# ishine/TargetDiarization

Hardware: AMD Instinct MI355X
Metric: real-time factor (audio-sec/wall-sec) full infer() pipe, 16kHz mono, 1/2/4/8 GPU (higher is better)
Workload: dtype f32 (split-f16 x3: fp32-accurate products from three f16 MFMA passes, fp32 accumulate); 1 GPU; BASELINE configs[3]: 1800 s synthetic conversation (two alternating speakers, 20 % overlap) = 180 x 10 s windows: MossFormer2 (90 windows per launch) -> loudness swap -> ERes2NetV2 on every 10 s window of both streams + cosine vs a target embedding -> Paraformer (SANM encoder, CIF predictor, NAR decoder, argmax tokens + timestamps) on 30 s segments of both streams -> CT-Transformer punctuation of ; windows_per_launch=90

## Files before the change

targetdiarization_amd/csrc/eres2net.hip:

```cpp
#include <hip/hip_runtime.h>

#include <algorithm>
#include <cmath>
#include <string>
#include <vector>

#include "../../include/tdx.h"
#include "gemm.hpp"
#include "gemm_h3.hpp"
#include "devutil.hpp"
#include "tdx_common.hpp"

using namespace tdx;

namespace {

constexpr int NSTAGE = 4, SCALE = 4, EMB = 192;
const int kBlocks[NSTAGE] = {3, 4, 6, 3};
const int kPlanes[NSTAGE] = {64, 128, 256, 512};
const int kStride[NSTAGE] = {1, 2, 2, 2};

inline size_t al(size_t n) { return (n + 63) / 64 * 64; }
inline int up(int n, int m) { return (n + m - 1) / m * m; }

// ... 77 lines not shown
    __device__ EpiNone row(int, int) const { return EpiNone{}; }
    __device__ void store(int z, int m, int n, float v, EpiNone, EpiNone) const { slab[(long)z * strideZ + (long)m * (int)ld + n] = v; }
};
__global__ __launch_bounds__(256) void slab_reduce_kernel(const float* __restrict__ slab, int nz, long MN, int N, const float* __restrict__ bias, float* __restrict__ out) {
    const long i = ((long)blockIdx.x * 256 + threadIdx.x) * 4;
    if (i >= MN) return;
    float4 a = *reinterpret_cast<const float4*>(slab + i);
    for (int z = 1; z < nz; ++z) {
        const float4 p = *reinterpret_cast<const float4*>(slab + (long)z * MN + i);
        a.x += p.x; a.y += p.y; a.z += p.z; a.w += p.w;
    }
    if (bias) { const float4 b = *reinterpret_cast<const float4*>(bias + (int)(i % N)); a.x += b.x; a.y += b.y; a.z += b.z; a.w += b.w; }
    *reinterpret_cast<float4*>(out + i) = a;
}
struct EpiChain {
    const float* b; float* cat; long ldcat; int coff; int width; int wpad;
    const float* o1; long ldo1; int next_off; float* spin;
    __device__ float col(int, int n) const { return b[n]; }
    __device__ EpiNone row(int, int) const { return EpiNone{}; }
    __device__ float aux(int, int m, int n, EpiNone) const { return (spin && n < width) ? o1[(long)m * (int)ldo1 + next_off + n] : 0.f; }
    __device__ void store(int, int m, int n, float v, EpiNone, float c, float nxt) const {
        if (n >= wpad) return;
        const float sp = relu20(v + c);
        if (n < width) cat[(long)m * (int)ldcat + coff + n] = sp;
        if (spin) spin[(long)m * wpad + n] = n < width ? sp + nxt : 0.f;
    }
};
struct EpiConv3 {
    const float* b; const float* res; float* out; long ld;
    __device__ float col(int, int n) const { return b[n]; }
    __device__ EpiNone row(int, int) const { return EpiNone{}; }
    __device__ float aux(int, int m, int n, EpiNone) const { return res[(long)m * (int)ld + n]; }
    __device__ void store(int, int m, int n, float v, EpiNone, float c, float r) const { out[(long)m * (int)ld + n] = relu20(v + c + r); }
};
struct EpiAffSilu {
    const float* b; float* t; int ipad;
    __device__ float col(int, int n) const { return b[n]; }
    __device__ EpiNone row(int, int) const { return EpiNone{}; }
    __device__ void store(int, int m, int n, float v, EpiNone, float c) const { if (n < ipad) t[(long)m * ipad + n] = siluf_acc(v + c); }
};
struct EpiAffGate {
    const float* b; const float* x; long ldx; const float* y; long ldy; float* out; long ldo; int C;
    __device__ float col(int, int n) const { return b[n]; }
    __device__ EpiNone row(int, int) const { return EpiNone{}; }
    __device__ float2 aux(int, int m, int n, EpiNone) const {
        return n < C ? make_float2(x[(long)m * (int)ldx + n], y[(long)m * (int)ldy + n]) : make_float2(0.f, 0.f);
    }
    __device__ void store(int, int m, int n, float v, EpiNone, float c, float2 xy) const {
        if (n >= C) return;
        const float att = 1.0f + tanhf(v + c);
        out[(long)m * (int)ldo + n] = xy.x * att + xy.y * (2.0f - att);
    }
};


struct ChainX3Args {
    const float* in; long ldin;
    const unsigned char* wp; const float* ws; int wk;
    int cinp;
    const float* b;
    float* cat; long ldcat; int coff;
    const float* o1; long ldo1; int next_off; float* spin; int ldspin;
    int H, W;
};
template <int CIN, int TH>
struct ChainX3Cfg {
// ... 529 lines not shown
                if (s < 1) { for (int j = 0; j < SCALE; ++j) jobs.push_back(&b.convs[j]); continue; }
                jobs.push_back(&b.conv1); if (b.has_sc) jobs.push_back(&b.sc);
                for (int j = 0; j < SCALE; ++j) jobs.push_back(&b.convs[j]);
                jobs.push_back(&b.conv3);
            }
        jobs.push_back(&h->ds);
        jobs.push_back(&h->fuse34.c0); jobs.push_back(&h->fuse34.c3);
        size_t bytes = 0;
        for (ConvW* c : jobs) bytes += (size_t)c->Npad * c->taps * c->cinp * 4 + al(c->Npad) * 4;
        e = hipMalloc(&h->dev_planes, bytes);
        if (e != hipSuccess) { hipFree(h->dev); delete h; return tdx::fail_hip(e, __FILE__, __LINE__); }
        unsigned char* q = h->dev_planes;
        for (ConvW* c : jobs) {
            const int K = c->taps * c->cinp;
            float* sc = (float*)(q + (size_t)c->Npad * K * 4);
            e = tdx::launch_h3_split_rows_long(h->dev + c->w, K, q, sc, c->Npad, K, nullptr);
            if (e != hipSuccess) { hipFree(h->dev_planes); hipFree(h->dev); delete h; return tdx::fail_hip(e, __FILE__, __LINE__); }
            c->hp = q; c->hs = sc;
            q += (size_t)c->Npad * K * 4 + al(c->Npad) * 4;
        }
        e = hipDeviceSynchronize();
        if (e != hipSuccess) { hipFree(h->dev_planes); hipFree(h->dev); delete h; return tdx::fail_hip(e, __FILE__, __LINE__); }
    }
    *out = h;
    return TDX_OK;
}

int tdx_eres2net_destroy(tdx_eres2net* h) {
    if (h) { if (h->dev_planes) hipFree(h->dev_planes); if (h->dev) hipFree(h->dev); delete h; }
    return TDX_OK;
}

namespace {
struct WsPlan { size_t P, keep3, o1, spin, tbuf, stats, hx, hcat, hin, slab, total; };
inline WsPlan ws_plan(const tdx_eres2net* h, int B, int F) {
    const Dims d = make_dims(F);
    WsPlan w{}; size_t mP = (size_t)B * 80 * F * 64, mo1 = 0, msp = 0, mt = 0, mhx = 0, mhc = 0, mhi = 0;
    int s = 0, cnt = 0;
    for (const BlockW& b : h->blocks) {
        const size_t rows = (size_t)B * d.H[s + 1] * d.W[s + 1];
        if (s >= 1) {
            const size_t rows_in = cnt == 0 ? (size_t)B * d.H[s] * d.W[s] : rows;
            mhx = std::max(mhx, rows_in * b.cin); mhc = std::max(mhc, rows * b.w4); mhi = std::max(mhi, rows * b.wpad);
        }
        mP = std::max(mP, rows * b.cout); mo1 = std::max(mo1, rows * b.w4); msp = std::max(msp, rows * b.wpad);
        if (b.is_aff) mt = std::max(mt, rows * (size_t)b.aff[0].ipad);
        if (++cnt == kBlocks[s]) { cnt = 0; ++s; }
    }
    const size_t rows3 = (size_t)B * d.H[3] * d.W[3], rows4 = (size_t)B * d.H[4] * d.W[4];
    mt = std::max(mt, rows4 * 512);
    w.P = al(mP + 4096); w.keep3 = al(rows3 * 1024 + 4096); w.o1 = al(mo1 + 4096); w.spin = al(msp + 4096); w.tbuf = al(mt + 4096);
    w.stats = al((size_t)B * 40960);
    mhx = std::max(mhx, rows3 * 1024);
    w.hx = al(mhx + 4096); w.hcat = al(mhc + 4096); w.hin = al(mhi + 4096);
    w.slab = rows4 <= (size_t)DS_SPLIT_ROWS ? al(DS_SPLIT * rows4 * 2048 + 4096) : 0;
    w.total = 3 * w.P + w.keep3 + 2 * w.o1 + 2 * w.spin + w.tbuf + w.stats + w.hx + w.hcat + w.hin + w.slab;
    return w;
}
}

size_t tdx_eres2net_workspace_bytes(const tdx_eres2net* h, int B, int F) {
    if (!h || B < 1 || F < 9) return 0;
    return ws_plan(h, B, F).total * sizeof(float);
}

double tdx_eres2net_flops(const tdx_eres2net* h, int B, int F) {
    if (!h || F < 1) return 0.0;
    const Dims d = make_dims(F);
    double fl = 2.0 * 80 * F * 9 * 64;
    int s = 0, cnt = 0;
    for (const BlockW& b : h->blocks) {
        const double pos = (double)d.H[s + 1] * d.W[s + 1];
        fl += 2.0 * pos * ((double)b.cin * b.w4 + 4.0 * 9 * b.width * b.width + (double)b.w4 * b.cout + (b.has_sc ? (double)b.cin * b.cout : 0.0));
        if (b.is_aff) fl += 3.0 * 2.0 * pos * (2.0 * b.width * (b.width / 4) + (double)(b.width / 4) * b.width);
        if (++cnt == kBlocks[s]) { cnt = 0; ++s; }
    }
    const double pos4 = (double)d.H[4] * d.W[4];
    fl += 2.0 * pos4 * (9.0 * 1024 * 2048 + 4096.0 * 512 + 512.0 * 2048) + 2.0 * 40960 * EMB;
    return fl * B;
}

int tdx_eres2net_forward(tdx_eres2net* h, const float* feat, int B, int F, float* emb, void* ws_, size_t ws_bytes, void* stream) {
    if (!h || !feat || !emb || !ws_ || B < 1) return tdx::fail(TDX_E_INVALID, "tdx_eres2net_forward: bad argument");
    if (F < 9) return tdx::fail(TDX_E_INVALID, "tdx_eres2net_forward: need >= 9 fbank frames (TSTP needs >= 2 pooled frames)");
    const WsPlan wp = ws_plan(h, B, F);
    if (ws_bytes < wp.total * sizeof(float)) return tdx::fail(TDX_E_WORKSPACE, "tdx_eres2net_forward: workspace too small");
    tdx::DeviceGuard guard(h->device);
    if (guard.err != hipSuccess) return tdx::fail_hip(guard.err, __FILE__, __LINE__);
    hipStream_t st = (hipStream_t)stream;
    const Dims d = make_dims(F);
    const size_t rows1 = (size_t)B * 80 * F;
    float* ws = (float*)ws_;
    float* P[3] = {ws, ws + wp.P, ws + 2 * wp.P};
    float* keep3 = ws + 3 * wp.P;
    float* o1 = keep3 + wp.keep3; float* cat = o1 + wp.o1;
    float* spin[2] = {cat + wp.o1, cat + wp.o1 + wp.spin};
    float* tbuf = spin[1] + wp.spin; float* stats = tbuf + wp.tbuf;
    unsigned char* hx = (unsigned char*)(stats + wp.stats);
    unsigned char* hcat = hx + wp.hx * sizeof(float);
    unsigned char* hin = hcat + wp.hcat * sizeof(float);
    float* slab = reinterpret_cast<float*>(hin + wp.hin * sizeof(float));
    const float* inv20 = h->dev + h->consts;
    const float* inv40 = h->dev + h->consts + 1;
    const unsigned char* zero_row = (const unsigned char*)(h->dev + h->consts + 64);

    hipLaunchKernelGGL(stem_kernel, dim3((unsigned)((rows1 * 16 + 255) / 256)), dim3(256), 0, st, feat, h->dev + h->stem_w, h->dev + h->stem_b, P[0], F, (long)rows1);
    LAUNCH_CHECK();
    const float* x = P[0];
    int cur = 0;
    int s = 0, cnt = 0;
    for (const BlockW& b : h->blocks) {
        const int Hin = (cnt == 0) ? d.H[s] : d.H[s + 1], Win = (cnt == 0) ? d.W[s] : d.W[s + 1];
        const int Ho = d.H[s + 1], Wo = d.W[s + 1];
        const long M = (long)B * Ho * Wo;
        const bool last_of_stage3 = (s == 2) && (cnt == kBlocks[2] - 1);
        const int iy = cur < 0 ? 0 : (cur + 1) % 3, ir = cur < 0 ? 1 : (cur + 2) % 3;
        float* y = last_of_stage3 ? keep3 : P[iy];
        float* res = P[ir];
        const bool x3 = b.conv1.hp != nullptr;
        const float* resid = x;
        if (x3) {
            int Hc = Hin, Wc = Win, sc_ = b.stride;
            if (b.stride == 2 && b.cin % 16 == 0) {
                const long R = (long)B * Ho * Wo;
                hipLaunchKernelGGL(split_rows_static_s2_kernel, dim3((unsigned)((R * (b.cin / 8) + 255) / 256)), dim3(256), 0, st,
                                   x, b.cin, hx, R, b.cin, Hin, Win, Ho, Wo, 1024.0f);
                LAUNCH_CHECK();
                Hc = Ho; Wc = Wo; sc_ = 1;
            } else if (tdx::launch_h3_split_rows_static(x, b.cin, hx, (long)B * Hin * Win, b.cin, 1024.0f, st) != hipSuccess)
                return tdx::fail_hip(hipGetLastError(), __FILE__, __LINE__);
            TRY(conv_gemm_h3(hx, inv20, zero_row, b.conv1, B, Hc, Wc, Ho, Wo, sc_, EpiRelu20{h->dev + b.conv1.b, o1, b.w4, b.w4}, st));
            if (b.has_sc) {
                TRY(conv_gemm_h3(hx, inv20, zero_row, b.sc, B, Hc, Wc, Ho, Wo, sc_, EpiBiasG{h->dev + b.sc.b, res, b.cout, b.cout}, st));
                resid = res;
            }
        } else {
            TRY(conv_gemm(x, b.cin, h->dev, b.conv1, B, Hin, Win, Ho, Wo, b.stride, EpiRelu20{h->dev + b.conv1.b, o1, b.w4, b.w4}, st));
            if (b.has_sc) {
                TRY(conv_gemm(x, b.cin, h->dev, b.sc, B, Hin, Win, Ho, Wo, b.stride, EpiBiasG{h->dev + b.sc.b, res, b.cout, b.cout}, st));
                resid = res;
            }
        }
        for (int j = 0; j < SCALE; ++j) {
            const float* in = j == 0 ? o1 : spin[j & 1];
            const long ldin = j == 0 ? b.w4 : b.wpad;
            const bool plain_next = (j + 1 < SCALE) && !b.is_aff;
            EpiChain e{h->dev + b.convs[j].b, cat, b.w4, j * b.width, b.width, b.wpad, o1, b.w4, (j + 1) * b.width,
                       plain_next ? spin[(j + 1) & 1] : nullptr};
            if (b.convs[j].hp && !b.is_aff && (b.width == 24 || b.width == 48)) {
                ChainX3Args ca{in, ldin, b.convs[j].hp, b.convs[j].hs, 9 * b.convs[j].cinp, b.convs[j].cinp, h->dev + b.convs[j].b, cat, b.w4, j * b.width,
                               o1, b.w4, (j + 1) * b.width, plain_next ? spin[(j + 1) & 1] : nullptr, b.wpad, Ho, Wo};
                if (b.width == 24) TRY((launch_chain_x3<24, 4>(ca, B, st)));
                else TRY((launch_chain_x3<48, 4>(ca, B, st)));
            } else if (x3) {
                if (tdx::launch_h3_split_rows_static(in, ldin, hin, M, b.wpad, 512.0f, st) != hipSuccess)
                    return tdx::fail_hip(hipGetLastError(), __FILE__, __LINE__);
                TRY(conv_gemm_h3(hin, inv40, zero_row, b.convs[j], B, Ho, Wo, Ho, Wo, 1, e, st));
            } else {
                TRY(conv_gemm(in, ldin, h->dev, b.convs[j], B, Ho, Wo, Ho, Wo, 1, e, st));
            }
            if (b.is_aff && j + 1 < SCALE)
                TRY(run_aff(h, b.aff[j], cat + j * b.width, b.w4, o1 + (j + 1) * b.width, b.w4, tbuf, spin[(j + 1) & 1], b.wpad, M, st));
        }
        if (x3) {
            if (tdx::launch_h3_split_rows_static(cat, b.w4, hcat, M, b.w4, 1024.0f, st) != hipSuccess)
                return tdx::fail_hip(hipGetLastError(), __FILE__, __LINE__);
            TRY(conv_gemm_h3(hcat, inv20, zero_row, b.conv3, B, Ho, Wo, Ho, Wo, 1, EpiConv3{h->dev + b.conv3.b, resid, y, b.cout}, st));
        } else {
            GemmArgs g = make_args((int)M, b.conv3.Npad, make_seg(cat, b.w4, h->dev + b.conv3.w, b.conv3.cinp, b.conv3.cinp));
            if (launch_gemm<false, false, false, false>(g, 1, EpiConv3{h->dev + b.conv3.b, resid, y, b.cout}, st) != hipSuccess)
                return tdx::fail_hip(hipGetLastError(), __FILE__, __LINE__);
        }
        x = y;
        cur = last_of_stage3 ? -1 : iy;
        if (++cnt == kBlocks[s]) { cnt = 0; ++s; }
    }
    const int i_ds = (cur + 1) % 3, i_fu = (cur + 2) % 3;
    const long M4 = (long)B * d.H[4] * d.W[4];
    if (tdx::launch_h3_split_rows_static(keep3, 1024, hx, (long)B * d.H[3] * d.W[3], 1024, 1024.0f, st) != hipSuccess)
        return tdx::fail_hip(hipGetLastError(), __FILE__, __LINE__);
    if (wp.slab && h->ds.taps == 9 && h->ds.Npad == 2048)
        TRY(conv_gemm_h3_tapsplit(hx, inv20, zero_row, h->ds, B, d.H[3], d.W[3], d.H[4], d.W[4], 2, slab, nullptr, P[i_ds], st));
    else
        TRY(conv_gemm_h3(hx, inv20, zero_row, h->ds, B, d.H[3], d.W[3], d.H[4], d.W[4], 2, EpiBiasG{nullptr, P[i_ds], 2048, 2048}, st));
    const char* aff34_env = getenv("TDX_ERES_AFF34_ROWS");
    const long aff34_min = aff34_env ? atol(aff34_env) : 8192;
    if (M4 >= aff34_min && 2 * M4 <= (long)B * 40960 && h->fuse34.c0.hp && h->fuse34.ipad == 512)
        TRY(run_aff34_x3(h, h->fuse34, x, P[i_ds], tbuf, P[i_fu], M4, hx, hcat, stats, hin, stats + M4, inv20, st));
    else
        TRY(run_aff(h, h->fuse34, x, 2048, P[i_ds], 2048, tbuf, P[i_fu], 2048, M4, st));
    hipLaunchKernelGGL(tstp_kernel, dim3(d.H[4], B), dim3(256), 0, st, P[i_fu], stats, d.W[4], 2048, d.H[4]);
    LAUNCH_CHECK();
    hipLaunchKernelGGL(seg_kernel, dim3(EMB, B), dim3(256), 0, st, stats, h->dev + h->seg_w, h->dev + h->seg_b, emb, 40960);
    LAUNCH_CHECK();
    return TDX_OK;
}

}
```

targetdiarization_amd/csrc/gemm_h3.hpp:

```cpp
#pragma once
#include <cstdio>
#include <cstdlib>
#include <typeinfo>
#include <vector>
#include <hip/hip_runtime.h>
#include <stdint.h>

#include "devutil.hpp"
#include "gemm.hpp"

namespace tdx {

typedef _Float16 f16x8 __attribute__((ext_vector_type(8)));

constexpr int H3_BM = 256, H3_BN = 256, H3_BK = 16, H3_THREADS = 512;
constexpr int H3_ROWB = 64;
constexpr int H3_OPER = 256 * H3_ROWB;
constexpr int H3_STAGE = 2 * H3_OPER;
constexpr int H3_NBUF = 4;
constexpr int H3_AUX_AHEAD = 3;
constexpr int H3_LDS = H3_NBUF * H3_STAGE;
constexpr int H3_LDS_EXTRA = 12288;

struct H3Seg {
// ... 223 lines not shown
    for (int j = 0; j < 4; ++j) { const _Float16 t = (_Float16)xs[j]; a[j] = t; b[j] = (_Float16)(xs[j] - (float)t); }
    H3Pair r;
    r.hi = __builtin_bit_cast(uint2, a); r.lo = __builtin_bit_cast(uint2, b);
    return r;
}
__device__ __forceinline__ uint4 h3_pair16(int q, float4 v, float s) {
    const H3Pair o = h3_split4(v, s);
    const bool odd = q & 1;
    const uint2 send = odd ? o.hi : o.lo;
    uint2 recv;
    recv.x = (unsigned)__builtin_amdgcn_mov_dpp((int)send.x, 0xB1, 0xF, 0xF, true);
    recv.y = (unsigned)__builtin_amdgcn_mov_dpp((int)send.y, 0xB1, 0xF, 0xF, true);
    return odd ? make_uint4(recv.x, recv.y, o.lo.x, o.lo.y) : make_uint4(o.hi.x, o.hi.y, recv.x, recv.y);
}
__device__ __forceinline__ void h3_emit4(unsigned char* prow, int q, float4 v, float s) {
    *reinterpret_cast<uint4*>(prow + (q >> 1) * 32 + ((q & 1) ? 16 : 0)) = h3_pair16(q, v, s);
}
__device__ __forceinline__ void h3_emit4_pred(unsigned char* prow, int q, float4 v, float s, bool ok) {
    const uint4 w = h3_pair16(q, v, s);
    if (ok) *reinterpret_cast<uint4*>(prow + (q >> 1) * 32 + ((q & 1) ? 16 : 0)) = w;
}
__device__ __forceinline__ float h3_wave_max(float v) {
    v = h3_row16_max(v);
    return fmaxf(fmaxf(h3_lane(v, 0), h3_lane(v, 16)), fmaxf(h3_lane(v, 32), h3_lane(v, 48)));
}
__device__ __forceinline__ float h3_absmax4(float4 v) { return fmaxf(fmaxf(fabsf(v.x), fabsf(v.y)), fmaxf(fabsf(v.z), fabsf(v.w))); }


struct H3PlOut { unsigned char* planes; long pitch; float* scale; float* ss; long seg_stride; };
template <class E, class = void> struct epi_has_plout { static constexpr bool value = false; };
template <class E> struct epi_has_plout<E, decltype((void)&E::plout, void())> { static constexpr bool value = true; };
template <class E, class = void> struct epi_has_rowout { static constexpr bool value = false; };
template <class E> struct epi_has_rowout<E, decltype((void)&E::rowout, void())> { static constexpr bool value = true; };
struct H3Conv {
    const float* w; int wld;
    int ncols;
    unsigned char* planes; long pitch;
    float sv;
    float* u32; int u0; long ld32;
    int S, Sp;
};
template <class E, class = void> struct epi_has_conv { static constexpr bool value = false; };
template <class E> struct epi_has_conv<E, decltype((void)&E::conv, void())> { static constexpr bool value = true; };
constexpr int H3_CONV_STEP = 240, H3_CONV_HALO = 8;
template <class T> __device__ __forceinline__ void h3_assume_row(const T&) {}
__device__ __forceinline__ void h3_assume_row(long rw) { __builtin_assume(rw >= 0); }

template <bool A_TR, bool B_TR, bool PAIRED, bool TWOSEG, class Epi, int VARIANT = 0, bool A_CONV = false>
__global__ __launch_bounds__(H3_THREADS, 2) void gemm_h3_kernel(H3Args g, Epi epi) {
    static_assert(!A_CONV || (!A_TR && !TWOSEG), "A_CONV: row-major A planes, one weight segment");
    constexpr bool PINGPONG = VARIANT == 5;
    extern __shared__ __attribute__((aligned(1024))) unsigned char lds[];
    const int tid = threadIdx.x;
    const int lane = tid & 63, wave = tid >> 6;
    const int l31 = lane & 31, h = lane >> 5;
    const int wm = wave >> 2, wn = wave & 3;

    int z, bm, bn;
    {
        const int x = blockIdx.x & 7, i = blockIdx.x >> 3;
        if (g.map_mode == 0) {
            z = blockIdx.y;
            int i2 = i, mbase = 0, mcur = g.mp;
            if (g.mc > 0) { const int tpc = g.mc * g.tiles_n, c = i / tpc; i2 = i - c * tpc; mbase = c * g.mc; mcur = min(g.mc, g.mp - mbase); }
            const int per = mcur * g.gw, ngf = g.tiles_n / g.gw;
            const int p = i2 / per;
// ... 560 lines not shown
            __syncthreads();
            H3_STAMP(3);
            const int hw = lane >> 5, l32 = lane & 31;
            unsigned char* const pbase = po.planes + (long)n0 * 4;
#pragma unroll 4
            for (int it = 0; it < 16; ++it) {
                const int rl = wave * 32 + it * 2 + hw;
                const int m = m0 + rl;
                const long pr = (!CHECK || m < g.M) ? epi.prow(z, min(m, g.M - 1)) : -1L;
                const f32x4 v4 = *reinterpret_cast<const f32x4*>(T + rl * 128 + ((4 * l32) ^ (((rl >> 2) & 1) << 5)));
                const float4 v = make_float4(v4[0], v4[1], v4[2], v4[3]);
                const float mu = h3_half_max(h3_absmax4(v));
                const float q2 = h3_half_sum((v.x * v.x + v.y * v.y) + (v.z * v.z + v.w * v.w));
                float inv;
                const float sc = h3_row_scale(mu, inv);
                h3_emit4_pred(pbase + (pr < 0 ? 0 : pr) * po.pitch, l32, v, sc, pr >= 0);
                if (l32 == 0 && pr >= 0) {
                    po.scale[(long)bn * po.seg_stride + pr] = inv;
                    if (po.ss) po.ss[(long)bn * po.seg_stride + pr] = q2;
                }
            }
        } else {
            int nn[2];
            decltype(epi.col(0, 0)) cc[2];
            float sc[2];
#pragma unroll
            for (int tn = 0; tn < 2; ++tn) {
                nn[tn] = n0 + tn * 128 + lcol;
                cc[tn] = epi.col(z, nn[tn]);
                sc[tn] = sb[(long)nn[tn] * sbm];
            }
            touch(cc[0]); touch(cc[1]); touch(sc[0]); touch(sc[1]);
            unsigned char* const pbase = po.planes + (long)n0 * 4;
            auto phase2 = [&](int hf) {
                __syncthreads();
#pragma unroll 4
                for (int it = 0; it < 16; ++it) {
                    const int rl = wave * 16 + it;
                    const int lr = (rl >> 6) * 128 + (2 * hf + ((rl >> 5) & 1)) * 32 + (rl & 31);
                    const int m = m0 + lr;
                    const long pr = (!CHECK || m < g.M) ? epi.prow(z, min(m, g.M - 1)) : -1L;
                    const f32x4 v4 = *reinterpret_cast<const f32x4*>(T + rl * 256 + ((4 * lane) ^ (((rl >> 2) & 1) << 5)));
                    const float4 v = make_float4(v4[0], v4[1], v4[2], v4[3]);
                    const float mu = h3_wave_max(h3_absmax4(v));
                    float q2 = (v.x * v.x + v.y * v.y) + (v.z * v.z + v.w * v.w);
                    if (po.ss) q2 = h3_wave_sum(q2);
                    float inv;
                    const float s_ = h3_row_scale(mu, inv);
                    if (pr >= 0) {
                        h3_emit4(pbase + pr * po.pitch, lane, v, s_);
                        if constexpr (epi_has_rowout<Epi>::value) *reinterpret_cast<f32x4*>(epi.rowout(z, pr, n0) + 4 * lane) = v4;
                        if (lane == 0) {
                            po.scale[(long)bn * po.seg_stride + pr] = inv;
                            if (po.ss) po.ss[(long)bn * po.seg_stride + pr] = q2;
                        }
                    }
                }
            };
            if constexpr (epi_has_aux<Epi>::value) {
                constexpr int AH = H3_AUX_AHEAD;
                decltype(epi.aux(0, 0, 0, RowT{})) ax[AH + 1][8];
                auto fetch = [&](int i, int set) {
                    const int tn = (i >> 2) & 1, tm = 2 * (i >> 3) + ((i >> 1) & 1), half = i & 1;
                    int lb = lrow + tm * 32;
                    asm volatile("" : "+v"(lb));
#pragma unroll
                    for (int r8 = 0; r8 < 8; ++r8) {
                        const int r = half * 8 + r8;
                        const int lr = lb + (r & 3) + 8 * (r >> 2);
                        ax[set][r8] = epi.aux(z, rowm(lr), nn[tn], row_of(lr));
                    }
                };
#pragma unroll
                for (int i = 0; i < AH; ++i) fetch(i, i % (AH + 1));
#pragma unroll
                for (int i = 0; i < 16; ++i) {
                    __builtin_amdgcn_sched_barrier(0);
                    if (i == 8) __syncthreads();
                    if (i + AH < 16) fetch(i + AH, (i + AH) % (AH + 1));
                    const int tn = (i >> 2) & 1, tmh = (i >> 1) & 1, tm = 2 * (i >> 3) + tmh, half = i & 1;
                    RowT rw[8];
                    float sr[8];
                    int lb = lrow + tm * 32;
                    asm volatile("" : "+v"(lb));
#pragma unroll
                    for (int r8 = 0; r8 < 8; ++r8) {
                        const int r = half * 8 + r8;
                        const int lr = lb + (r & 3) + 8 * (r >> 2);
// ... 385 lines not shown
```

targetdiarization_amd/csrc/mf2.hip:

```cpp
#include <hip/hip_runtime.h>

#include <algorithm>
#include <cmath>
#include <cstdio>
#include <cstring>
#include <map>
#include <mutex>
#include <string>
#include <vector>

#include "../../include/tdx.h"
#include "gemm.hpp"
#include "gemm_x6.hpp"
#include "gemm_h3.hpp"
#include "gemm_h3a.hpp"
#include "mf2_kernels.hpp"
#include "tdx_common.hpp"

using namespace tdx;

namespace {

constexpr int C = 512, HID = 2048, QK = 128, HQ = HID + QK, INNER = 256;

// ... 109 lines not shown
    __device__ bool full(int z, int m0) const { return (z % G) * 256 + m0 + 256 <= S; }
    __device__ int2 aux(int z, int m, int c, long) const {
        const int b = z / G, s = min((z % G) * 256 + m, S - 1);
        const int c2 = c & ~1;
        const unsigned char* p = vuP + (long)b * Sp * (8L * E) + (long)s * (8 * E) + (c2 >> 5) * 128 + (c2 & 31) * 2 + (c & 1) * 64;
        return make_int2(*reinterpret_cast<const int*>(p), __float_as_int(u32[((long)b * S + s) * E + c]));
    }
    __device__ float2 pairmul(float k) const { return make_float2(-1.4426950408889634f, k); }
    __device__ float val2_scaled(int, int, int c, float av, float au, long rw, float, int2 w) const {
        typedef _Float16 h2 __attribute__((ext_vector_type(2)));
        const unsigned ov = (unsigned)__builtin_amdgcn_mov_dpp(w.x, 0xB1, 0xF, 0xF, true);
        const unsigned sel = (c & 1) ? 0x03020706u : 0x05040100u;
        const h2 pv = __builtin_bit_cast(h2, __builtin_amdgcn_perm(ov, (unsigned)w.x, sel));
        const float vs = (float)pv[0] + (float)pv[1];
        const float t0 = au * vs;
        const float t1 = av * __int_as_float(w.y);
        const float o = t0 * __builtin_amdgcn_rcpf(1.0f + __builtin_amdgcn_exp2f(t1));
        return rw < 0 ? 0.f : o;
    }
    __device__ tdx::H3PlOut plout(int) const { return tdx::H3PlOut{oP, 4L * E, os, oss, M}; }
    __device__ long prow(int z, int m) const { return row(z, m); }
};
struct EpiBiasPrelu {
    const float* b; const float* a; float* out; long ld;
    __device__ Col2 col(int, int n) const { return Col2{b[n], a[0]}; }
    __device__ EpiNone row(int, int) const { return EpiNone{}; }
    __device__ void store(int, int m, int n, float v, EpiNone, Col2 c) const {
        v += c.a;
        out[(long)m * (int)ld + n] = v >= 0.f ? v : c.b * v;
    }
    __device__ float* ptr(int, int m, int n) const { return out + (long)m * (int)ld + n; }
    __device__ long ldm() const { return ld; }
    __device__ void put(float* p, float v, EpiNone, Col2 c) const { v += c.a; *p = v >= 0.f ? v : c.b * v; }
};
struct EpiBiasSilu { const float* b; float* out; long ld;
    __device__ float col(int, int n) const { return b[n]; }
    __device__ EpiNone row(int, int) const { return EpiNone{}; }
    __device__ void store(int, int m, int n, float v, EpiNone, float c) const { out[(long)m * (int)ld + n] = siluf_acc(v + c); }
    __device__ float* ptr(int, int m, int n) const { return out + (long)m * (int)ld + n; }
    __device__ long ldm() const { return ld; }
    __device__ void put(float* p, float v, EpiNone, float c) const { *p = siluf_acc(v + c); } };
struct EpiBiasRelu { const float* b; float* out; long ld;
    __device__ float col(int, int n) const { return b[n]; }
    __device__ EpiNone row(int, int) const { return EpiNone{}; }
    __device__ void store(int, int m, int n, float v, EpiNone, float c) const { out[(long)m * (int)ld + n] = fmaxf(v + c, 0.f); }
    __device__ float* ptr(int, int m, int n) const { return out + (long)m * (int)ld + n; }
    __device__ long ldm() const { return ld; }
    __device__ void put(float* p, float v, EpiNone, float c) const { *p = fmaxf(v + c, 0.f); } };
struct EpiBiasReluPl { const float* b; unsigned char* P; float* sc;
    __device__ float col(int, int n) const { return b[n]; }
    __device__ EpiNone row(int, int) const { return EpiNone{}; }
    __device__ float val(int, int, int, float v, EpiNone, float c) const { return fmaxf(v + c, 0.f); }
    __device__ tdx::H3PlOut plout(int) const { return tdx::H3PlOut{P, 1024, sc, nullptr, 0}; }
    __device__ long prow(int, int m) const { return m; } };
struct EpiBias { const float* b; float* out; long ld;
    __device__ float col(int, int n) const { return b ? b[n] : 0.f; }
    __device__ EpiNone row(int, int) const { return EpiNone{}; }
    __device__ void store(int, int m, int n, float v, EpiNone, float c) const { out[(long)m * (int)ld + n] = v + c; }
    __device__ float* ptr(int, int m, int n) const { return out + (long)m * (int)ld + n; }
    __device__ long ldm() const { return ld; }
    __device__ void put(float* p, float v, EpiNone, float c) const { *p = v + c; } };
struct EpiBiasHalves { const float* b; float* out; long M;
    __device__ float col(int, int n) const { return b[n]; }
    __device__ EpiNone row(int, int) const { return EpiNone{}; }
    __device__ void store(int, int m, int n, float v, EpiNone, float c) const { out[(long)(n >> 9) * M * C + (long)m * C + (n & 511)] = v + c; } };
struct EpiBiasResidual { const float* b; float* x; long ld;
// ... 127 lines not shown
        auto it = side_ctx.find(st);
        if (it != side_ctx.end()) return &it->second;
        if (side_ctx.size() >= MAX_SIDE_CTX) return nullptr;
        hipStreamCaptureStatus cs = hipStreamCaptureStatusNone;
        if (hipStreamIsCapturing(st, &cs) != hipSuccess) { (void)hipGetLastError(); return nullptr; }
        if (cs != hipStreamCaptureStatusNone) return nullptr;
        SideCtx c;
        if (hipStreamCreateWithFlags(&c.side, hipStreamNonBlocking) != hipSuccess ||
            hipEventCreateWithFlags(&c.ev_fork, hipEventDisableTiming) != hipSuccess ||
            hipEventCreateWithFlags(&c.ev_heads, hipEventDisableTiming) != hipSuccess ||
            hipEventCreateWithFlags(&c.ev_sim, hipEventDisableTiming) != hipSuccess) {
            (void)hipGetLastError();
            if (c.ev_sim) hipEventDestroy(c.ev_sim);
            if (c.ev_heads) hipEventDestroy(c.ev_heads);
            if (c.ev_fork) hipEventDestroy(c.ev_fork);
            if (c.side) hipStreamDestroy(c.side);
            return nullptr;
        }
        return &(side_ctx[st] = c);
    }
};

namespace {

struct Plan {
    int B, T, S, G, Sp, splits, kchunk, nblk_enc, nblk_gn, nchunk1, nchunk2;
    long M;
    size_t fs, xp, xs, xss, os, oss, zrow, E, z, x, rs, hid, vu, qk4, Abuf, slab, kvu, o, t, hraw, h, hp, hs, vuP, AbufP, Asc, qks, KvuP, kvus, uvpre, uv, f, p, c1, c2, pe, rc, rsn, stat,
        part, tap0, tap1, mask, hdr, total;
};

inline size_t al(size_t n) { return (n + 63) / 64 * 64; }

bool make_plan(const tdx_mf2* h, int B, int T, Plan& P) {
    if (B < 1 || T < 16) return false;
    P.B = B; P.T = T; P.S = (T - 16) / 8 + 1; P.G = (P.S + 255) / 256; P.Sp = P.G * 256; P.M = (long)B * P.S;
    int sp = (1536 + 16 * B - 1) / (16 * B); if (sp < 1) sp = 1;
    int maxsp = (P.S + 511) / 512; if (sp > maxsp) sp = maxsp;
    P.splits = sp;
    P.kchunk = ((P.S + sp - 1) / sp + 31) / 32 * 32;
    P.splits = (P.S + P.kchunk - 1) / P.kchunk;
    P.nblk_enc = (P.S + ENC_TOK - 1) / ENC_TOK;
    P.nblk_gn = (P.S + 63) / 64;
    const int ts = ddn_ts(B, P.S);
    P.nchunk1 = (P.S + ts - 1) / ts;
    P.nchunk2 = 2 * ((P.S + 2 * ts - 1) / (2 * ts));
    const size_t M = (size_t)P.M;
    size_t off = 0;
    auto take = [&](size_t n) { size_t o = off; off += al(n); return o; };
    P.E = take(M * C); P.z = take(M * C); P.x = take(M * C); P.rs = take(M);
    P.hid = take(M * HQ); P.vu = take(M * HID);
    P.qk4 = take((size_t)4 * B * P.Sp * QK);
    P.Abuf = take((size_t)B * P.G * 65536);
    P.slab = take((size_t)B * P.splits * QK * HID);
    P.kvu = take((size_t)B * QK * HID);
    P.o = take(M * 1024); P.t = take(M * C);
    P.hraw = take(M * INNER); P.h = take(M * INNER);
    P.hp = take(M * 1024);
    P.hs = take(2 * M);
    P.vuP = take((size_t)B * P.Sp * HID);
    P.AbufP = take((size_t)B * P.G * 65536);
    P.Asc = take((size_t)B * P.Sp);
    P.qks = take((size_t)3 * B * P.Sp);
    P.KvuP = take((size_t)B * QK * HID);
    P.kvus = take((size_t)B + (size_t)B * (QK * HID / 1024) + 64);
    P.uvpre = take(M * C); P.uv = take(M * C); P.f = take(M * INNER); P.fs = take(M); P.p = take(M * INNER);
    P.xp = take(M * C);
    P.xs = take(2 * M); P.xss = take(2 * M);
    P.os = take(8 * M); P.oss = take(8 * M);
    P.zrow = take(1024);
    P.c1 = take(M * INNER); P.c2 = take(M * INNER);
    P.pe = take((size_t)P.S * C); P.rc = take((size_t)P.S * 16); P.rsn = take((size_t)P.S * 16);
    P.stat = take((size_t)B * 2 + (size_t)2 * B * 256 * 2 + 64);
    size_t npart = (size_t)B * (P.nblk_enc > P.nblk_gn ? P.nblk_enc : P.nblk_gn) * 2;
    size_t npart_in = (size_t)B * (P.nchunk1 > P.nchunk2 ? P.nchunk1 : P.nchunk2) * 256 * 2;
    if (npart_in > npart) npart = npart_in;
    P.part = take(npart * 2);
    if (h->taps) { P.tap0 = take(M * C); P.tap1 = take(M * C); P.mask = take(2 * M * C); P.hdr = take((size_t)h->L * 2 + 64); }
    else { P.tap0 = P.tap1 = P.mask = P.hdr = 0; }
    P.total = off;
    return true;
}

#define LAUNCH_CHECK()                                    \
    do {                                                  \
        hipError_t e__ = hipGetLastError();               \
        if (e__ != hipSuccess) return tdx::fail_hip(e__, __FILE__, __LINE__); \
    } while (0)

inline dim3 rows4(long M) { return dim3((unsigned)((M + 3) / 4)); }
// ... 613 lines not shown
            q.hp = (unsigned char*)qk4; q.hs = qks; q.sv = w.sv_lk; q.silu_in = 1;
            TRY(launch_conv17<3>(q, B, sq));
            if (hdr) {
                hipLaunchKernelGGL(planes_absmax_kernel, dim3(1024), dim3(256), 0, st, reinterpret_cast<const _Float16*>(vuP), (long)B * Sp * HID * 2, hdr + 2 * l);
                LAUNCH_CHECK();
                hipLaunchKernelGGL(planes_absmax_kernel, dim3(256), dim3(256), 0, sq, reinterpret_cast<const _Float16*>(qk4) + 3L * B * Sp * 256, (long)B * Sp * 256,
                                   hdr + 2 * l + 1);
                LAUNCH_CHECK();
            }
            if (fork && hipEventRecord(sc->ev_heads, sc->side) != hipSuccess) return tdx::fail_hip(hipGetLastError(), __FILE__, __LINE__);
        }
        TRY(attention_core_h3((const unsigned char*)qk4, qks, vuP, nullptr, w.st, B, S, 1024, P.splits, P.kchunk, Abuf, AbufP, Asc, slab, kvu, KvuP,
                              kvus, nullptr, nullptr, nullptr, st, oP, os, oss, fork ? sc->side : nullptr, fork ? sc->ev_heads : nullptr, fork ? sc->ev_sim : nullptr, vu));
        {
            tdx::H3Args g{};
            g.seg[0] = tdx::h3_seg(oP, os, 4L * 1024, w.hWo.p, w.hWo.s, 4L * 1024, 1024);
            g.seg[0].segk = 128; g.seg[0].strideSeg = M;
            g.nseg = 1; g.M = (int)M; g.N = C;
            EpiHiddenSN<8, false> e{oss, M, S, 0.03125f, w.go, w.bo, t, C};
            if (launch_linear_x3<false>(g, e, st) != hipSuccess) return tdx::fail_hip(hipGetLastError(), __FILE__, __LINE__);
        }
        {
            Conv17Args a{};
            a.in = t; a.ld_in = C; a.col0 = 0; a.wT = w.cw_o; a.C = C; a.out = x; a.ld_out = C; a.S = S; a.Sp = Sp; a.silu_in = 1;
            a.xp = xp; a.xs = xs; a.xs_stride = M;
            TRY(launch_conv17<1>(a, B, st));
        }
        if (h->taps && l == 0) hipMemcpyAsync(ws + P.tap0, x, M * C * sizeof(float), hipMemcpyDeviceToDevice, st);
        {
            tdx::H3Args g{};
            g.seg[0] = tdx::h3_seg(xp, xs, 4L * C, w.hW1.p, w.hW1.s, 4L * C, C);
            g.seg[0].segk = 256; g.seg[0].strideSeg = M;
            g.nseg = 1; g.M = (int)M; g.N = INNER;
            if (tdx::launch_gemm_h3x<false, false, false, false>(g, 1, EpiBiasPrelu{w.b1, w.a1, hraw, INNER}, st) != hipSuccess)
                return tdx::fail_hip(hipGetLastError(), __FILE__, __LINE__);
        }
        hipLaunchKernelGGL((layernorm_kernel<INNER, true>), rows4(M), dim3(256), 0, st, hraw, w.ln1g, w.ln1b, hh, (float*)nullptr, M, 1e-5f,
                           hp, hs);
        LAUNCH_CHECK();
        TRY(linear_h3(hp, hs, (int)M, w.hWuv, C, INNER, EpiBiasSilu{w.buv, uvpre, C}, st));
        {
            Conv17Args a{};
            a.in = uvpre; a.ld_in = C; a.col0 = 0; a.wT = w.cw_uv; a.C = C; a.out = uv; a.ld_out = C; a.S = S; a.Sp = Sp;
            a.xp = hp; a.xs = hs;
            TRY(launch_conv17<0>(a, B, st));
        }
        TRY(linear_h3(hp, hs, (int)M, w.hWl, INNER, INNER, EpiBiasReluPl{w.bl, fP, fs}, st));
        TRY(linear_h3(fP, fs, (int)M, w.hWp, INNER, INNER, EpiBias{nullptr, p, INNER}, st));
        TRY(ddn_core(p, B, S, w.w1T, w.w2T, w.ing, w.inb, w.pre, c1, c2, stat1, stat2, part, st));
        hipLaunchKernelGGL(fsmn_tail_kernel, rows4(M), dim3(256), 0, st, c2, stat2, w.ing + INNER, w.inb + INNER, w.pre + INNER, uv, hh,
                           w.ln2g, w.ln2b, hp, hs, M, S);
        LAUNCH_CHECK();
        TRY(linear_h3(hp, hs, (int)M, w.hW2, C, INNER, EpiBiasResidualPl{w.b2, x, C, xp, xs, xss, M}, st));
        if (h->taps && l == 0) hipMemcpyAsync(ws + P.tap1, x, M * C * sizeof(float), hipMemcpyDeviceToDevice, st);
    }

    hipLaunchKernelGGL((layernorm_kernel<C, false>), rows4(M), dim3(256), 0, st, x, h->lnfg, h->lnfb, t, (float*)nullptr, M, 1e-6f);
    LAUNCH_CHECK();
    hipLaunchKernelGGL(rowblock_stats_kernel, dim3(P.nblk_gn, B), dim3(256), 0, st, t, part, S, 64, P.nblk_gn);
    LAUNCH_CHECK();
    hipLaunchKernelGGL(gn_finalize_kernel, dim3(B), dim3(64), 0, st, part, gnstat, P.nblk_gn, (double)S * C, 1e-8);
    LAUNCH_CHECK();
    float* r = uvpre;
    hipLaunchKernelGGL((gn_apply_kernel<1>), dim3((unsigned)((M * 128 + 255) / 256)), dim3(256), 0, st, t, gnstat, h->gn2g, h->gn2b, z,
                       h->prelu, r, M, S);
    LAUNCH_CHECK();
    float* r2 = o;
    TRY(split_linear_h3(r, C, hp, hs, (int)M, h->hWout, 2 * C, C, EpiBiasHalves{h->bout, r2, M}, st));
    float* gate = vu;
    {
        if (tdx::launch_h3_split_rows(r2, C, hp, hs, 2 * M, C, st) != hipSuccess) return tdx::fail_hip(hipGetLastError(), __FILE__, __LINE__);
        tdx::H3Args g{};
// ... 181 lines not shown
```

Before: 493.9 audio-s/s.

## Fuse split-plane emission into GEMM epilogues for ERes2Net conv3 and MossFormer LN

Extends the h3 GEMM plane-output epilogue so it can take either a static plane scale or a per-row transform hook. ERes2Net conv3 now writes the f16 split planes for the next block's conv1 (or the stage-3 downsample input) directly, which skips a separate split-rows pass. MossFormer2's first FFN GEMM now applies PReLU, then LayerNorm, then the plane split inside the epilogue using wave reductions, which removes the hraw buffer and a layernorm launch. Both paths sit behind environment toggles that default on. The risks are extra epilogue work and register pressure, and the LN fusion assumes one wave spans the full INNER row.

```diff
diff --git a/targetdiarization_amd/csrc/eres2net.hip b/targetdiarization_amd/csrc/eres2net.hip
--- a/targetdiarization_amd/csrc/eres2net.hip
+++ b/targetdiarization_amd/csrc/eres2net.hip
@@ -133,6 +133,17 @@
     __device__ EpiNone row(int, int) const { return EpiNone{}; }
     __device__ float aux(int, int m, int n, EpiNone) const { return res[(long)m * (int)ld + n]; }
     __device__ void store(int, int m, int n, float v, EpiNone, float c, float r) const { out[(long)m * (int)ld + n] = relu20(v + c + r); }
+};
+struct EpiConv3Pl {
+    const float* b; const float* res; float* out; long ld; unsigned char* P;
+    __device__ float col(int, int n) const { return b[n]; }
+    __device__ EpiNone row(int, int) const { return EpiNone{}; }
+    __device__ float aux(int, int m, int n, EpiNone) const { return res[(long)m * (int)ld + n]; }
+    __device__ float val(int, int, int, float v, EpiNone, float c, float r) const { return relu20(v + c + r); }
+    __device__ float* rowout(int, long m, int n0) const { return out + m * ld + n0; }
+    __device__ float plstatic() const { return 1024.0f; }
+    __device__ tdx::H3PlOut plout(int) const { return tdx::H3PlOut{P, 4 * ld, nullptr, nullptr, 0}; }
+    __device__ long prow(int, int m) const { return m; }
 };
 struct EpiAffSilu {
     const float* b; float* t; int ipad;
@@ -728,7 +739,11 @@
 }
 
 namespace {
-struct WsPlan { size_t P, keep3, o1, spin, tbuf, stats, hx, hcat, hin, slab, total; };
+struct WsPlan { size_t P, keep3, o1, spin, tbuf, stats, hx, hcat, hin, slab, hk3, total; };
+inline bool fuse_hx() {
+    static const bool on = [] { const char* e = getenv("TDX_FUSE_HX"); return e ? atoi(e) != 0 : true; }();
+    return on;
+}
 inline WsPlan ws_plan(const tdx_eres2net* h, int B, int F) {
     const Dims d = make_dims(F);
     WsPlan w{}; size_t mP = (size_t)B * 80 * F * 64, mo1 = 0, msp = 0, mt = 0, mhx = 0, mhc = 0, mhi = 0;
@@ -750,7 +765,8 @@
     mhx = std::max(mhx, rows3 * 1024);
     w.hx = al(mhx + 4096); w.hcat = al(mhc + 4096); w.hin = al(mhi + 4096);
     w.slab = rows4 <= (size_t)DS_SPLIT_ROWS ? al(DS_SPLIT * rows4 * 2048 + 4096) : 0;
-    w.total = 3 * w.P + w.keep3 + 2 * w.o1 + 2 * w.spin + w.tbuf + w.stats + w.hx + w.hcat + w.hin + w.slab;
+    w.hk3 = fuse_hx() ? al(rows3 * 1024 + 4096) : 0;
+    w.total = 3 * w.P + w.keep3 + 2 * w.o1 + 2 * w.spin + w.tbuf + w.stats + w.hx + w.hcat + w.hin + w.slab + w.hk3;
     return w;
 }
 }
@@ -796,6 +812,7 @@
     unsigned char* hcat = hx + wp.hx * sizeof(float);
     unsigned char* hin = hcat + wp.hcat * sizeof(float);
     float* slab = reinterpret_cast<float*>(hin + wp.hin * sizeof(float));
+    unsigned char* hk3 = reinterpret_cast<unsigned char*>(slab + wp.slab);
     const float* inv20 = h->dev + h->consts;
     const float* inv40 = h->dev + h->consts + 1;
     const unsigned char* zero_row = (const unsigned char*)(h->dev + h->consts + 64);
@@ -805,6 +822,9 @@
     const float* x = P[0];
     int cur = 0;
     int s = 0, cnt = 0;
+    bool hk3_ready = false;
+    bool hx_ready = false;
+    size_t bi = 0;
     for (const BlockW& b : h->blocks) {
         const int Hin = (cnt == 0) ? d.H[s] : d.H[s + 1], Win = (cnt == 0) ? d.W[s] : d.W[s + 1];
         const int Ho = d.H[s + 1], Wo = d.W[s + 1];
@@ -823,6 +843,7 @@
                                    x, b.cin, hx, R, b.cin, Hin, Win, Ho, Wo, 1024.0f);
                 LAUNCH_CHECK();
                 Hc = Ho; Wc = Wo; sc_ = 1;
+            } else if (hx_ready) {
             } else if (tdx::launch_h3_split_rows_static(x, b.cin, hx, (long)B * Hin * Win, b.cin, 1024.0f, st) != hipSuccess)
                 return tdx::fail_hip(hipGetLastError(), __FILE__, __LINE__);
             TRY(conv_gemm_h3(hx, inv20, zero_row, b.conv1, B, Hc, Wc, Ho, Wo, sc_, EpiRelu20{h->dev + b.conv1.b, o1, b.w4, b.w4}, st));
@@ -861,8 +882,19 @@
         if (x3) {
             if (tdx::launch_h3_split_rows_static(cat, b.w4, hcat, M, b.w4, 1024.0f, st) != hipSuccess)
                 return tdx::fail_hip(hipGetLastError(), __FILE__, __LINE__);
-            TRY(conv_gemm_h3(hcat, inv20, zero_row, b.conv3, B, Ho, Wo, Ho, Wo, 1, EpiConv3{h->dev + b.conv3.b, resid, y, b.cout}, st));
+            const BlockW* nx = bi + 1 < h->blocks.size() ? &h->blocks[bi + 1] : nullptr;
+            const bool to_next = nx && cnt + 1 < kBlocks[s] && nx->stride == 1 && nx->conv1.hp != nullptr && nx->cin == b.cout;
+            hx_ready = false;
+            if (fuse_hx() && (to_next || last_of_stage3) && b.cout % 256 == 0) {
+                TRY(conv_gemm_h3(hcat, inv20, zero_row, b.conv3, B, Ho, Wo, Ho, Wo, 1,
+                                 EpiConv3Pl{h->dev + b.conv3.b, resid, y, b.cout, last_of_stage3 ? hk3 : hx}, st));
+                hx_ready = to_next;
+                if (last_of_stage3) hk3_ready = true;
+            } else {
+                TRY(conv_gemm_h3(hcat, inv20, zero_row, b.conv3, B, Ho, Wo, Ho, Wo, 1, EpiConv3{h->dev + b.conv3.b, resid, y, b.cout}, st));
+            }
         } else {
+            hx_ready = false;
             GemmArgs g = make_args((int)M, b.conv3.Npad, make_seg(cat, b.w4, h->dev + b.conv3.w, b.conv3.cinp, b.conv3.cinp));
             if (launch_gemm<false, false, false, false>(g, 1, EpiConv3{h->dev + b.conv3.b, resid, y, b.cout}, st) != hipSuccess)
                 return tdx::fail_hip(hipGetLastError(), __FILE__, __LINE__);
@@ -870,15 +902,18 @@
         x = y;
         cur = last_of_stage3 ? -1 : iy;
         if (++cnt == kBlocks[s]) { cnt = 0; ++s; }
+        ++bi;
     }
     const int i_ds = (cur + 1) % 3, i_fu = (cur + 2) % 3;
     const long M4 = (long)B * d.H[4] * d.W[4];
-    if (tdx::launch_h3_split_rows_static(keep3, 1024, hx, (long)B * d.H[3] * d.W[3], 1024, 1024.0f, st) != hipSuccess)
+    const unsigned char* ds_in = hx;
+    if (hk3_ready) ds_in = hk3;
+    else if (tdx::launch_h3_split_rows_static(keep3, 1024, hx, (long)B * d.H[3] * d.W[3], 1024, 1024.0f, st) != hipSuccess)
         return tdx::fail_hip(hipGetLastError(), __FILE__, __LINE__);
     if (wp.slab && h->ds.taps == 9 && h->ds.Npad == 2048)
-        TRY(conv_gemm_h3_tapsplit(hx, inv20, zero_row, h->ds, B, d.H[3], d.W[3], d.H[4], d.W[4], 2, slab, nullptr, P[i_ds], st));
+        TRY(conv_gemm_h3_tapsplit(ds_in, inv20, zero_row, h->ds, B, d.H[3], d.W[3], d.H[4], d.W[4], 2, slab, nullptr, P[i_ds], st));
     else
-        TRY(conv_gemm_h3(hx, inv20, zero_row, h->ds, B, d.H[3], d.W[3], d.H[4], d.W[4], 2, EpiBiasG{nullptr, P[i_ds], 2048, 2048}, st));
+        TRY(conv_gemm_h3(ds_in, inv20, zero_row, h->ds, B, d.H[3], d.W[3], d.H[4], d.W[4], 2, EpiBiasG{nullptr, P[i_ds], 2048, 2048}, st));
     const char* aff34_env = getenv("TDX_ERES_AFF34_ROWS");
     const long aff34_min = aff34_env ? atol(aff34_env) : 8192;
     if (M4 >= aff34_min && 2 * M4 <= (long)B * 40960 && h->fuse34.c0.hp && h->fuse34.ipad == 512)
diff --git a/targetdiarization_amd/csrc/gemm_h3.hpp b/targetdiarization_amd/csrc/gemm_h3.hpp
--- a/targetdiarization_amd/csrc/gemm_h3.hpp
+++ b/targetdiarization_amd/csrc/gemm_h3.hpp
@@ -279,6 +279,10 @@
 template <class E> struct epi_has_plout<E, decltype((void)&E::plout, void())> { static constexpr bool value = true; };
 template <class E, class = void> struct epi_has_rowout { static constexpr bool value = false; };
 template <class E> struct epi_has_rowout<E, decltype((void)&E::rowout, void())> { static constexpr bool value = true; };
+template <class E, class = void> struct epi_has_rowfn { static constexpr bool value = false; };
+template <class E> struct epi_has_rowfn<E, decltype((void)&E::rowfn, void())> { static constexpr bool value = true; };
+template <class E, class = void> struct epi_has_plstatic { static constexpr bool value = false; };
+template <class E> struct epi_has_plstatic<E, decltype((void)&E::plstatic, void())> { static constexpr bool value = true; };
 struct H3Conv {
     const float* w; int wld;
     int ncols;
@@ -905,6 +909,8 @@
             }
             touch(cc[0]); touch(cc[1]); touch(sc[0]); touch(sc[1]);
             unsigned char* const pbase = po.planes + (long)n0 * 4;
+            auto rctx = [&] { if constexpr (epi_has_rowfn<Epi>::value) return epi.rowprep(z, n0, lane); else return EpiNone{}; }();
+            touch(rctx);
             auto phase2 = [&](int hf) {
                 __syncthreads();
 #pragma unroll 4
@@ -914,6 +920,19 @@
                     const int m = m0 + lr;
                     const long pr = (!CHECK || m < g.M) ? epi.prow(z, min(m, g.M - 1)) : -1L;
                     const f32x4 v4 = *reinterpret_cast<const f32x4*>(T + rl * 256 + ((4 * lane) ^ (((rl >> 2) & 1) << 5)));
+                    if constexpr (epi_has_rowfn<Epi>::value || epi_has_plstatic<Epi>::value) {
+                        float4 v = make_float4(v4[0], v4[1], v4[2], v4[3]);
+                        float4 vo = v;
+                        if constexpr (epi_has_rowfn<Epi>::value) vo = epi.rowfn(rctx, v);
+                        float inv = 0.f, s_;
+                        if constexpr (epi_has_plstatic<Epi>::value) s_ = epi.plstatic();
+                        else s_ = h3_row_scale(h3_wave_max(h3_absmax4(v)), inv);
+                        if (pr >= 0) {
+                            h3_emit4(pbase + pr * po.pitch, lane, v, s_);
+                            if constexpr (epi_has_rowout<Epi>::value) *reinterpret_cast<f32x4*>(epi.rowout(z, pr, n0) + 4 * lane) = f32x4{vo.x, vo.y, vo.z, vo.w};
+                            if constexpr (!epi_has_plstatic<Epi>::value) { if (lane == 0) po.scale[(long)bn * po.seg_stride + pr] = inv; }
+                        }
+                    } else {
                     const float4 v = make_float4(v4[0], v4[1], v4[2], v4[3]);
                     const float mu = h3_wave_max(h3_absmax4(v));
                     float q2 = (v.x * v.x + v.y * v.y) + (v.z * v.z + v.w * v.w);
@@ -927,6 +946,7 @@
                             po.scale[(long)bn * po.seg_stride + pr] = inv;
                             if (po.ss) po.ss[(long)bn * po.seg_stride + pr] = q2;
                         }
+                    }
                     }
                 }
             };
diff --git a/targetdiarization_amd/csrc/mf2.hip b/targetdiarization_amd/csrc/mf2.hip
--- a/targetdiarization_amd/csrc/mf2.hip
+++ b/targetdiarization_amd/csrc/mf2.hip
@@ -165,6 +165,33 @@
     __device__ float* ptr(int, int m, int n) const { return out + (long)m * (int)ld + n; }
     __device__ long ldm() const { return ld; }
     __device__ void put(float* p, float v, EpiNone, Col2 c) const { v += c.a; *p = v >= 0.f ? v : c.b * v; }
+};
+struct EpiBiasPreluLN {
+    const float* b; const float* a; const float* g1; const float* b1; float* hh; unsigned char* hp; float* hs;
+    struct Ctx { float4 g, b; };
+    __device__ Col2 col(int, int n) const { return Col2{b[n], a[0]}; }
+    __device__ EpiNone row(int, int) const { return EpiNone{}; }
+    __device__ float val(int, int, int, float v, EpiNone, Col2 c) const { v += c.a; return v >= 0.f ? v : c.b * v; }
+    __device__ Ctx rowprep(int, int n0, int lane) const {
+        return Ctx{*reinterpret_cast<const float4*>(g1 + n0 + 4 * lane), *reinterpret_cast<const float4*>(b1 + n0 + 4 * lane)};
+    }
+    __device__ float4 rowfn(const Ctx& c, float4& v) const {
+        constexpr float eps = 1e-5f;
+        const float mean = wave_sum((v.x + v.y) + (v.z + v.w)) * (1.0f / INNER);
+        v.x -= mean; v.y -= mean; v.z -= mean; v.w -= mean;
+        const float rstd = 1.0f / sqrtf(wave_sum((v.x * v.x + v.y * v.y) + (v.z * v.z + v.w * v.w)) * (1.0f / INNER) + eps);
+        v.x = v.x * rstd * c.g.x + c.b.x; v.y = v.y * rstd * c.g.y + c.b.y;
+        v.z = v.z * rstd * c.g.z + c.b.z; v.w = v.w * rstd * c.g.w + c.b.w;
+        const float4 out = v;
+        const float mean2 = wave_sum((v.x + v.y) + (v.z + v.w)) * (1.0f / INNER);
+        v.x -= mean2; v.y -= mean2; v.z -= mean2; v.w -= mean2;
+        const float rstd2 = 1.0f / sqrtf(wave_sum((v.x * v.x + v.y * v.y) + (v.z * v.z + v.w * v.w)) * (1.0f / INNER) + eps);
+        v.x *= rstd2; v.y *= rstd2; v.z *= rstd2; v.w *= rstd2;
+        return out;
+    }
+    __device__ float* rowout(int, long m, int n0) const { return hh + m * INNER + n0; }
+    __device__ tdx::H3PlOut plout(int) const { return tdx::H3PlOut{hp, 4L * INNER, hs, nullptr, 0}; }
+    __device__ long prow(int, int m) const { return m; }
 };
 struct EpiBiasSilu { const float* b; float* out; long ld;
     __device__ float col(int, int n) const { return b[n]; }
@@ -358,6 +385,11 @@
 
 inline size_t al(size_t n) { return (n + 63) / 64 * 64; }
 
+inline bool fuse_ln() {
+    static const bool on = [] { const char* e = getenv("TDX_FUSE_LN"); return e ? atoi(e) != 0 : true; }();
+    return on;
+}
+
 bool make_plan(const tdx_mf2* h, int B, int T, Plan& P) {
     if (B < 1 || T < 16) return false;
     P.B = B; P.T = T; P.S = (T - 16) / 8 + 1; P.G = (P.S + 255) / 256; P.Sp = P.G * 256; P.M = (long)B * P.S;
@@ -381,7 +413,8 @@
     P.slab = take((size_t)B * P.splits * QK * HID);
     P.kvu = take((size_t)B * QK * HID);
     P.o = take(M * 1024); P.t = take(M * C);
-    P.hraw = take(M * INNER); P.h = take(M * INNER);
+    P.hraw = fuse_ln() ? 0 : take(M * INNER);
+    P.h = take(M * INNER);
     P.hp = take(M * 1024);
     P.hs = take(2 * M);
     P.vuP = take((size_t)B * P.Sp * HID);
@@ -1061,12 +1094,17 @@
             g.seg[0] = tdx::h3_seg(xp, xs, 4L * C, w.hW1.p, w.hW1.s, 4L * C, C);
             g.seg[0].segk = 256; g.seg[0].strideSeg = M;
             g.nseg = 1; g.M = (int)M; g.N = INNER;
-            if (tdx::launch_gemm_h3x<false, false, false, false>(g, 1, EpiBiasPrelu{w.b1, w.a1, hraw, INNER}, st) != hipSuccess)
-                return tdx::fail_hip(hipGetLastError(), __FILE__, __LINE__);
-        }
-        hipLaunchKernelGGL((layernorm_kernel<INNER, true>), rows4(M), dim3(256), 0, st, hraw, w.ln1g, w.ln1b, hh, (float*)nullptr, M, 1e-5f,
-                           hp, hs);
-        LAUNCH_CHECK();
+            if (fuse_ln()) {
+                if (tdx::launch_gemm_h3x<false, false, false, false>(g, 1, EpiBiasPreluLN{w.b1, w.a1, w.ln1g, w.ln1b, hh, hp, hs}, st) != hipSuccess)
+                    return tdx::fail_hip(hipGetLastError(), __FILE__, __LINE__);
+            } else {
+                if (tdx::launch_gemm_h3x<false, false, false, false>(g, 1, EpiBiasPrelu{w.b1, w.a1, hraw, INNER}, st) != hipSuccess)
+                    return tdx::fail_hip(hipGetLastError(), __FILE__, __LINE__);
+                hipLaunchKernelGGL((layernorm_kernel<INNER, true>), rows4(M), dim3(256), 0, st, hraw, w.ln1g, w.ln1b, hh, (float*)nullptr, M, 1e-5f,
+                                   hp, hs);
+                LAUNCH_CHECK();
+            }
+        }
         TRY(linear_h3(hp, hs, (int)M, w.hWuv, C, INNER, EpiBiasSilu{w.buv, uvpre, C}, st));
         {
             Conv17Args a{};
```

Result: faster. 501.4 audio-s/s, median of 6 (+1.5%).
